# stockeh/swift

Measured on AMD Instinct MI355X. Metric: 6h forecast steps/sec (members x ICs) on 128x256x69 ERA5, higher is better.
Workload: dtype bf16

## Files before the change

### include/swiftk.h

```cpp
#ifndef SWIFTK_H
#define SWIFTK_H

#include <stdint.h>

#ifdef __cplusplus
extern "C" {
#endif

#define SWIFTK_F32 0
#define SWIFTK_BF16 1
#define SWIFTK_BF16X3 2

#define SWIFTK_EINVAL (-1)
#define SWIFTK_ESHAPE (-2)
#define SWIFTK_EALIGN (-3)
#define SWIFTK_EWORKSPACE (-4)

#define SWIFTK_EPI_NONE 0
#define SWIFTK_EPI_BIAS_POS 1
#define SWIFTK_EPI_SWIGLU 2
#define SWIFTK_EPI_QKNORM 3
#define SWIFTK_EPI_SWIGLU_BOTH 6
#define SWIFTK_EPI_SWIGLU_BWD 7
#define SWIFTK_EPI_ACCUM 5
// ... 44 lines not shown
int swiftk_modnorm_residual_pair_slabs_bf16(const void* y_slabs, int64_t ldy, int64_t slab_stride, void* x_hi, int64_t ldh, void* x_lo,
                                            int64_t ldl, int lo_bits, const float* gamma, const float* beta, const float* mod,
                                            int64_t ldmod, int64_t M, int d, int64_t rows_per_sample, float eps, void* stream);
int swiftk_modnorm_residual_pair_halves_bf16(const void* y_slabs, int64_t slab_stride, const int64_t* tail, void* x_hi, int64_t ldh,
                                             void* x_lo, const float* gamma, const float* beta, const float* mod, int64_t ldmod,
                                             int64_t M, int d, int64_t rows_per_sample, float eps, void* stream);
int swiftk_gemm_modnorm_residual_pair(const void* A, int64_t lda, const void* W, int64_t ldw, int64_t K, void* x_hi, int64_t ldh,
                                      void* x_lo, int64_t ldl, const float* gamma, const float* beta, const float* mod,
                                      int64_t ldmod, int64_t M, int d, int64_t rows_per_sample, float eps,
                                      int rows_per_workgroup, void* stream);
int swiftk_split_pair(const float* src, int64_t lds, void* hi, int64_t ldh, void* lo, int64_t ldl, int lo_bits, int64_t rows,
                      int64_t cols, void* stream);
int swiftk_gemm_bias_pos_pair(const void* A, int64_t lda, const void* W, int64_t ldw, void* hi, int64_t ldh, void* lo, int64_t ldl,
                              int64_t M, int64_t N, int64_t K, const float* bias, const float* pos, int64_t pos_rows, void* stream);

int swiftk_patchify(const float* src0, int c0, float s0, const float* src1, int c1, float s1, const float* src2, int c2,
                    float s2, void* A, int64_t lda, int B, int H, int W, int p1, int p2, int dtype, void* stream);
int swiftk_patchify_scaled(const float* src0, int c0, float s0, const float* s0_per_sample, const float* src1, int c1, float s1,
                           const float* src2, int c2, float s2, void* A, int64_t lda, int B, int H, int W, int p1, int p2,
                           int dtype, void* stream);

int swiftk_unpatchify_affine(const float* tok, int64_t ldt, const float* xt, const float* alpha, const float* beta,
                             float* out, int B, int C, int H, int W, int p1, int p2, void* stream);

int swiftk_timestep_embed(const float* t, const float* aux, const float* freqs, const float* aux_w, const float* aux_b,
                          float* emb, int B, int d, int aux_dim, float timestep_weight, void* stream);

int swiftk_linear_small(const float* x, int64_t ldx, const float* W, int64_t ldw, const float* bias, float* out,
                        int64_t ldo, int B, int N, int K, int act, void* stream);

int swiftk_unit_noise(float* out, const int64_t* seeds, const int64_t* step_dev, int64_t step_add, int B,
                      int64_t n_per_unit, int mode, void* stream);
int swiftk_counter_add(int64_t* counter, int64_t value, void* stream);

int swiftk_rollout_update(float* xstd, const float* y, float* phys, const float* mx, const float* sx, const float* st,
                          int B, int C, int64_t hw, void* stream);

int swiftk_unit_checksum(const float* x, double* out, double* scratch, int B, int64_t n, void* stream);

int swiftk_axpby(float* out, float a, const float* x, float b, const float* y, int64_t n, void* stream);

int swiftk_zero_f32(float* p, int64_t n, void* stream);
int swiftk_zero_check_report(unsigned long long* out26);

#define SWIFTK_PROF_ATTENTION 100
int swiftk_profile_gemm(int epilogue, int64_t N);
// ... 227 lines not shown
```

### swift_amd/_lib.py

```python
from __future__ import annotations

import ctypes as C
import os
from typing import Optional

_HERE = os.path.dirname(os.path.abspath(__file__))
LIB_PATH = os.environ.get("SWIFTK_LIB") or os.path.join(_HERE, "csrc", "libswiftk.so")

F32, BF16 = 0, 1
BF16X3 = 2
EPI_NONE, EPI_BIAS_POS, EPI_SWIGLU, EPI_QKNORM, EPI_ACCUM, EPI_SWIGLU_BOTH, EPI_SWIGLU_BWD = 0, 1, 2, 3, 5, 6, 7
EPI_QKNORM_JVP, EPI_SWIGLU_JVP = 8, 9
EPI_SWIGLU_SPLIT3 = 10
ATTN_PRENORM, ATTN_NO_PIPE, ATTN_TILED = 1, 2, 4
PROF_ATTENTION = 100

_ERR = {-1: "SWIFTK_EINVAL (bad argument)", -2: "SWIFTK_ESHAPE (unsupported shape)",
        -3: "SWIFTK_EALIGN (misaligned pointer / leading dimension)", -4: "SWIFTK_EWORKSPACE (workspace too small)"}


class SwiftkError(RuntimeError):
    pass


# ... 44 lines not shown
        + [("layers_host", C.POINTER(Layer))]
        + [("head_dim", C.c_int32)]
    )


_p, _i, _l, _f = C.c_void_p, C.c_int, C.c_int64, C.c_float
_SIGS = {
    "swiftk_version": ([], C.c_int),
    "swiftk_gemm_k_pad": ([_i, _l], _l),
    "swiftk_gemm": ([_p, _l, _p, _l, _p, _l, _l, _l, _l, _i, _i, _i, _p, _p, _l, _p], _i),
    "swiftk_gemm_chunked": ([_p, _l, _p, _l, _p, _l, _l, _l, _l, _i, _i, _i, _p, _p, _l, _i, _p, _l, _p], _i),
    "swiftk_gemm_chunk_scratch_bytes": ([], _l),
    "swiftk_window_attention": ([_p, _l, _p, _l, _p, _i, _i, _i, _i, _i, _i, _i, _i, _i, _p], _i),
    "swiftk_modnorm_residual": ([_p, _l, _p, _p, _l, _p, _p, _p, _l, _l, _i, _l, _f, _i, _p], _i),
    "swiftk_modnorm_residual_pair": ([_p, _l, _p, _l, _p, _l, _i, _p, _p, _p, _l, _l, _i, _l, _f, _p], _i),
    "swiftk_modnorm_residual_pair_to": ([_p, _l, _p, _p, _l, _p, _l, _i, _p, _p, _p, _l, _l, _i, _l, _f, _p], _i),
    "swiftk_modnorm_residual_pair_slabs": ([_p, _l, _l, _p, _l, _p, _l, _i, _p, _p, _p, _l, _l, _i, _l, _f, _p], _i),
    "swiftk_split_pair": ([_p, _l, _p, _l, _p, _l, _i, _l, _l, _p], _i),
    "swiftk_unit_noise": ([_p, _p, _p, _l, _i, _l, _i, _p], _i),
    "swiftk_counter_add": ([_p, _l, _p], _i),
    "swiftk_patchify": ([_p, _i, _f, _p, _i, _f, _p, _i, _f, _p, _l, _i, _i, _i, _i, _i, _i, _p], _i),
    "swiftk_patchify_scaled": ([_p, _i, _f, _p, _p, _i, _f, _p, _i, _f, _p, _l, _i, _i, _i, _i, _i, _i, _p], _i),
    "swiftk_unpatchify_affine": ([_p, _l, _p, _p, _p, _p, _i, _i, _i, _i, _i, _i, _p], _i),
    "swiftk_timestep_embed": ([_p, _p, _p, _p, _p, _p, _i, _i, _i, _f, _p], _i),
    "swiftk_linear_small": ([_p, _l, _p, _l, _p, _p, _l, _i, _i, _i, _i, _p], _i),
    "swiftk_rollout_update": ([_p, _p, _p, _p, _p, _p, _i, _i, _l, _p], _i),
    "swiftk_cast_pad": ([_p, _l, _p, _l, _l, _l, _i, _p], _i),
    "swiftk_split3": ([_p, _l, _p, _l, _l, _l, _i, _p], _i),
    "swiftk_axpby": ([_p, _f, _p, _f, _p, _l, _p], _i),
    "swiftk_zero_f32": ([_p, _l, _p], _i),
    "swiftk_modnorm_residual_split3": ([_p, _l, _p, _p, _l, _p, _l, _p, _p, _p, _l, _l, _i, _l, _f, _p], _i),
    "swiftk_zero_check_report": ([_p], _i),
    "swiftk_unit_checksum": ([_p, _p, _p, _i, _l, _p], _i),
    "swiftk_timestep_embed_jvp": ([_p, _p, _p, _p, _i, _i, _f, _p], _i),
    "swiftk_silu_jvp": ([_p, _p, _p, _p, _l, _p], _i),
    "swiftk_qknorm_jvp": ([_p, _p, _l, _p, _p, _l, _i, _i, _i, _p], _i),
    "swiftk_window_attention_jvp": ([_p, _p, _l, _p, _p, _l, _i, _i, _i, _i, _i, _i, _i, _i, _p], _i),
    "swiftk_modnorm_jvp": ([_p, _p, _l, _p, _p, _p, _p, _l, _p, _p, _p, _p, _l, _l, _i, _l, _f, _i, _p], _i),
    "swiftk_modnorm_jvp_pair": ([_p, _p, _l, _p, _p, _p, _p, _l, _p, _p, _p, _p, _p, _p, _l, _l, _i, _l, _f, _p], _i),
    "swiftk_swiglu_jvp": ([_p, _p, _l, _p, _p, _l, _l, _i, _i, _p], _i),
    "swiftk_gemm_bias_pos_pair": ([_p, _l, _p, _l, _p, _l, _p, _l, _l, _l, _l, _p, _p, _l, _p], _i),
    "swiftk_gemm_splitk_bf16": ([_p, _l, _p, _l, _p, _l, _l, _l, _l, _l, _i, _p], _i),
    "swiftk_gemm_tail_split_bf16": ([_p, _l, _p, _l, _p, _l, _l, _l, _l, _l, _p, _p], _i),
    "swiftk_modnorm_residual_pair_halves_bf16": ([_p, _l, _p, _p, _l, _p, _p, _p, _p, _l, _l, _i, _l, _f, _p], _i),
    "swiftk_modnorm_residual_pair_slabs_bf16": ([_p, _l, _l, _p, _l, _p, _l, _i, _p, _p, _p, _l, _l, _i, _l, _f, _p], _i),
    "swiftk_embed_bwd_sums": ([_p, _l, _p, _p, _p, _l, _l, _i, _l, _p], _i),
# ... 72 lines not shown
```

### swift_amd/csrc/common.h

```cpp
#pragma once
#include <hip/hip_runtime.h>
#include <stdint.h>

#include "../../include/swiftk.h"

typedef __attribute__((ext_vector_type(8))) __bf16 bf16x8;
typedef __attribute__((ext_vector_type(4))) float f32x4;
typedef __attribute__((ext_vector_type(16))) float f32x16;
typedef __attribute__((ext_vector_type(4))) short s16x4;
typedef uint16_t bf16_t;

#define LDS_PTR(p) ((__attribute__((address_space(3))) void*)(p))
#define GLB_PTR(p) ((const __attribute__((address_space(1))) void*)(p))

#define SWIFTK_CHECK_LAUNCH()                         \
    do {                                              \
        hipError_t e__ = hipGetLastError();           \
        if (e__ != hipSuccess) return (int)e__;       \
    } while (0)

__device__ __forceinline__ bf16_t f2bf(float f) {
    __bf16 b = (__bf16)f;
    return __builtin_bit_cast(bf16_t, b);
}
// ... 134 lines not shown
int swiftk_zero_f32_impl(float* p, int64_t n, void* stream, int who);
extern int g_zero_memset;
int swiftk_zero_check_enable();
int swiftk_zero_check_launch(const float* p, int64_t n, void* stream);

bool swiftk_prof_begin(int kind, int n, hipStream_t st);
void swiftk_prof_end(hipStream_t st);
extern int g_fwd_tiled;
extern int g_fwd_fused;
extern int g_x3_exact;
extern int g_fwd_pair;
extern int g_f32_chunk_k;
extern int g_fwd_splitk;
extern int g_attn_bwd_pipe;
extern int g_attn_bwd_fuse;
extern int g_modnorm_bwd_fused;
extern int g_modnorm_jvp_rows;
extern int g_x3_ffsplit;
extern int g_x3_normsplit;
extern int g_x3_qkonly;
extern int g_x3_attnpv;
extern int g_fwd_tail;
extern int g_fwd_pepair;
extern int g_modnorm_nt;
extern int g_persist_wgs;
extern int g_fwd_rownorm;
extern int g_rownorm_dbg;
extern int g_tn_pp;
extern int g_attn_pp;
extern int g_attn_sl;
extern int g_attn_dbg;
```

### swift_amd/csrc/elementwise.hip

```cpp
#include "common.h"
#include <type_traits>

int g_modnorm_nt = 3;

namespace {

__device__ __forceinline__ void load8_nt(const float* p, float (&v)[8]) {
    typedef __attribute__((ext_vector_type(4))) float v4;
    const v4 a = __builtin_nontemporal_load(reinterpret_cast<const v4*>(p));
    const v4 b = __builtin_nontemporal_load(reinterpret_cast<const v4*>(p + 4));
    v[0] = a[0]; v[1] = a[1]; v[2] = a[2]; v[3] = a[3]; v[4] = b[0]; v[5] = b[1]; v[6] = b[2]; v[7] = b[3];
}
__device__ __forceinline__ void store8_nt(float* p, const float (&v)[8]) {
    typedef __attribute__((ext_vector_type(4))) float v4;
    __builtin_nontemporal_store(v4{v[0], v[1], v[2], v[3]}, reinterpret_cast<v4*>(p));
    __builtin_nontemporal_store(v4{v[4], v[5], v[6], v[7]}, reinterpret_cast<v4*>(p + 4));
}

template <typename T, int SLOTS>
__global__ __launch_bounds__(256) void modnorm_kernel(const T* __restrict__ y, int64_t ldy, float* __restrict__ x,
                                                      T* __restrict__ xc, int64_t ldc, const float* __restrict__ gamma,
                                                      const float* __restrict__ beta, const float* __restrict__ mod,
                                                      int64_t ldmod, int64_t M, int d, int64_t rps, float eps, int nt_x) {
    const bool NT_X = nt_x != 0;
// ... 650 lines not shown
    const int F = a.p1 * a.p2 * a.C;
    const int cpr = (int)(a.lda >> 3);
    const int64_t tok0 = ((int64_t)b * a.gh + gy) * a.gw + gxb * 16;
    for (int i = tid; i < 16 * cpr; i += 256) {
        const int tk = i / cpr, fc = i - tk * cpr;
        float v[8];
        int f = 8 * fc;
        int pp = f / a.C, c = f - pp * a.C;
#pragma unroll
        for (int e = 0; e < 8; ++e) {
            float val = 0.f;
            if (f < F) {
                const int i1 = pp / a.p2, i2 = pp - i1 * a.p2;
                val = ptile[(c * a.p1 + i1) * rs + tk * a.p2 + i2];
            }
            v[e] = val;
            ++f;
            if (++c == a.C) { c = 0; ++pp; }
        }
        store8<T>(A + (tok0 + tk) * a.lda + 8 * fc, v);
    }
}

__global__ __launch_bounds__(256) void unpatchify_kernel(const float* __restrict__ tok, int64_t ldt,
                                                         const float* __restrict__ xt, const float* __restrict__ alpha,
                                                         const float* __restrict__ beta, float* __restrict__ out, int B,
                                                         int C, int H, int W, int p1, int p2) {
    const int64_t total = (int64_t)B * C * H * W;
    const int gw = W / p2, gh = H / p1;
    for (int64_t i = (int64_t)blockIdx.x * 256 + threadIdx.x; i < total; i += (int64_t)gridDim.x * 256) {
        const int xw = (int)(i % W);
        int64_t r = i / W;
        const int yh = (int)(r % H);
        r /= H;
        const int c = (int)(r % C);
        const int64_t b = r / C;
        const int gy = yh / p1, i1 = yh - gy * p1, gx = xw / p2, i2 = xw - gx * p2;
        const float f = tok[(b * gh * gw + (int64_t)gy * gw + gx) * ldt + (c * p1 + i1) * p2 + i2];
        const float bb = beta ? beta[b] : 1.0f;
        float o = bb * f;
        if (xt) o = (alpha ? alpha[b] : 0.0f) * xt[i] + o;
        out[i] = o;
    }
}

__global__ __launch_bounds__(256) void unpatchify4_kernel(const float* __restrict__ tok, int64_t ldt,
// ... 517 lines not shown

extern "C" int swiftk_patchify_scaled(const float* src0, int c0, float s0, const float* s0_per_sample, const float* src1, int c1,
                                      float s1, const float* src2, int c2, float s2, void* A, int64_t lda, int B, int H, int W,
                                      int p1, int p2, int dtype, void* stream) {
    if (!A || !src0 || c0 <= 0 || c1 < 0 || c2 < 0 || B <= 0 || p1 <= 0 || p2 <= 0) return SWIFTK_EINVAL;
    if ((c1 > 0 && !src1) || (c2 > 0 && !src2)) return SWIFTK_EINVAL;
    if (H % p1 || W % p2) return SWIFTK_ESHAPE;
    PatchArgs a;
    a.src[0] = src0; a.src[1] = src1 ? src1 : src0; a.src[2] = src2 ? src2 : src0;
    a.cn[0] = c0; a.cn[1] = c1; a.cn[2] = c2;
    a.c0[0] = 0; a.c0[1] = c0; a.c0[2] = c0 + c1;
    if (c1 == 0) a.c0[1] = 1 << 30;
    if (c2 == 0) a.c0[2] = 1 << 30;
    a.sc[0] = s0; a.sc[1] = s1; a.sc[2] = s2;
    a.sc0 = s0_per_sample;
    a.B = B; a.H = H; a.W = W; a.p1 = p1; a.p2 = p2; a.C = c0 + c1 + c2; a.gh = H / p1; a.gw = W / p2;
    a.lda = lda;
    if (lda < (int64_t)p1 * p2 * a.C) return SWIFTK_ESHAPE;
    hipStream_t st = static_cast<hipStream_t>(stream);
    const int rs = 16 * p2 + 4;
    const size_t tile_bytes = (size_t)a.C * p1 * rs * sizeof(float);
    bool aligned = !(a.gw & 15) && !((16 * p2) & 3) && !(W & 3) && !(lda & 7) && !((uintptr_t)A & 15) && tile_bytes <= 64 * 1024;
    for (int k = 0; k < 3; ++k) aligned = aligned && !((uintptr_t)a.src[k] & 15);
    if (aligned && (dtype == SWIFTK_BF16 || dtype == SWIFTK_F32)) {
        const dim3 grid(a.gw / 16, a.gh, B);
        if (dtype == SWIFTK_BF16)
            hipLaunchKernelGGL(patchify_tiled_kernel<bf16_t>, grid, dim3(256), tile_bytes, st, a, static_cast<bf16_t*>(A), rs);
        else
            hipLaunchKernelGGL(patchify_tiled_kernel<float>, grid, dim3(256), tile_bytes, st, a, static_cast<float*>(A), rs);
        SWIFTK_CHECK_LAUNCH();
        return 0;
    }
    const int grid = grid_for((int64_t)B * a.gh * a.gw * lda);
    if (dtype == SWIFTK_BF16)
        hipLaunchKernelGGL(patchify_kernel<bf16_t>, dim3(grid), dim3(256), 0, st, a, static_cast<bf16_t*>(A));
    else if (dtype == SWIFTK_F32)
        hipLaunchKernelGGL(patchify_kernel<float>, dim3(grid), dim3(256), 0, st, a, static_cast<float*>(A));
    else
        return SWIFTK_EINVAL;
    SWIFTK_CHECK_LAUNCH();
    return 0;
}

extern "C" int swiftk_patchify(const float* src0, int c0, float s0, const float* src1, int c1, float s1, const float* src2,
                               int c2, float s2, void* A, int64_t lda, int B, int H, int W, int p1, int p2, int dtype,
                               void* stream) {
// ... 231 lines not shown
```

### swift_amd/csrc/forward.hip

```cpp
#include "common.h"

#include <algorithm>

int g_fwd_tiled = 1;
int g_x3_exact = 17;
int g_fwd_pair = 2;
int g_f32_chunk_k = 256;
int g_fwd_splitk = 2;
int g_fwd_tail = 3;
int g_fwd_pepair = 1;
int g_x3_attnpv = 1;
int g_x3_qkonly = 2;
int g_x3_ffsplit = 1;
int g_fwd_fused = 1;

namespace {

__global__ __launch_bounds__(256) void zero_cols_kernel(char* p, int64_t ld_b, int64_t col0_b, int64_t ncol_b, int64_t rows) {
    const int64_t per = ncol_b >> 2, total = rows * per;
    for (int64_t i = (int64_t)blockIdx.x * 256 + threadIdx.x; i < total; i += (int64_t)gridDim.x * 256) {
        const int64_t r = i / per, c = i - r * per;
        *reinterpret_cast<uint32_t*>(p + r * ld_b + col0_b + 4 * c) = 0u;
    }
}

struct Layout {
    int64_t emb, h1, lat, mod, ape, x, xt, xlo, qkv, att, y, yslab, hmid, tok, kscr, a3, a3h, total;
};

inline int64_t al(int64_t v) { return (v + 255) & ~(int64_t)255; }

bool model_ok(const swiftk_model* m) {
    if (!m || !m->layers_host) return false;
    if (m->dtype != SWIFTK_F32 && m->dtype != SWIFTK_BF16 && m->dtype != SWIFTK_BF16X3) return false;
    if (m->depth <= 0 || m->dim <= 0 || m->heads <= 0 || m->head_dim < 0 || (m->head_dim == 0 && m->dim % m->heads)) return false;
    if (m->H % m->p1 || m->W % m->p2) return false;
// ... 300 lines not shown
            if (halves_norm)
                RUN(swiftk_modnorm_residual_pair_halves_bf16(yslab, SS, nullptr, xT, m->kd, xlo, ly.ln2_g, ly.ln2_b,
                                                             mod + (int64_t)(2 * i + 1) * 2 * d, ldmod, M, d, ntok, 1e-6f, stream));
            else
            RUN(swiftk_modnorm_residual_pair_slabs_bf16(yslab, d, SS, xT, m->kd, xlo, d, lo_bits, ly.ln2_g, ly.ln2_b,
                                                        mod + (int64_t)(2 * i + 1) * 2 * d, ldmod, M, d, ntok, 1e-6f, stream));
            continue;
        }
        if (splitk) {
            RUN(swiftk_gemm_splitk(hmid, m->kmlp, ly.w2_w, m->kmlp, yslab, d, M * d, M, d, m->kmlp, SWIFTK_BF16, 2, stream));
            RUN(swiftk_modnorm_residual_pair_slabs(yslab, d, M * d, xT, m->kd, xlo, d, lo_bits, ly.ln2_g, ly.ln2_b,
                                                   mod + (int64_t)(2 * i + 1) * 2 * d, ldmod, M, d, ntok, 1e-6f, stream));
            continue;
        }
        RUN(G(hmid, m->kmlp, ly.w2_w, y, d, d, m->kmlp, m->mlp, dt, SWIFTK_EPI_NONE, nullptr, nullptr, 0, (x3_exact & 8) != 0));
        if (pair)
            RUN(swiftk_modnorm_residual_pair(y, d, xT, m->kd, xlo, d, lo_bits, ly.ln2_g, ly.ln2_b, mod + (int64_t)(2 * i + 1) * 2 * d, ldmod,
                                             M, d, ntok, 1e-6f, stream));
        else
            RUN(NORM(y, ly.ln2_g, ly.ln2_b, mod + (int64_t)(2 * i + 1) * 2 * d, true));
    }

    const int po4 = (m->out_ch * m->p1 * m->p2 + 3) & ~3;
    RUN(G(xT, m->kd, m->head_w, tok, po4, po4, kdv, d, SWIFTK_F32, SWIFTK_EPI_NONE, nullptr, nullptr, 0, (x3_exact & 32) != 0));
    RUN(swiftk_unpatchify_affine(tok, po4, xt, alpha, beta, out, B, m->out_ch, m->H, m->W, m->p1, m->p2, stream));
    return 0;
}

extern "C" int swiftk_swinv2_forward(const swiftk_model* m, const float* src0, int c0, float s0, const float* src1, int c1,
                                     float s1, const float* src2, int c2, float s2, const float* t, const float* aux,
                                     const float* xt, const float* alpha, const float* beta, float* out, float* logvar,
                                     int B, void* workspace, int64_t workspace_bytes, void* stream) {
    return swiftk_swinv2_forward_scaled(m, src0, c0, s0, nullptr, src1, c1, s1, src2, c2, s2, t, aux, xt, alpha, beta, out, logvar,
                                        B, workspace, workspace_bytes, stream);
}
```

### swift_amd/csrc/gemm.hip

```cpp
#include "common.h"

int g_persist_wgs = 256;

namespace {

template <typename OutT>
__device__ __forceinline__ float swiglu_out(float g, float u) {
    if constexpr (sizeof(OutT) == 4) return g / (1.0f + expf(-g)) * u;
    else return g * __builtin_amdgcn_rcpf(1.0f + __expf(-g)) * u;
}

constexpr int BM = 256;
constexpr int BN = 352;
constexpr int ROWB = 128;
constexpr int A_BYTES = BM * ROWB;
constexpr int B_BYTES = BN * ROWB;
constexpr int STAGE = A_BYTES + B_BYTES;
constexpr int LDS_BYTES = 2 * STAGE;
constexpr int NT = 512;
constexpr int A_PIECES = A_BYTES / 1024;
constexpr int B_PIECES = B_BYTES / 1024;
constexpr int MI = 4, NI = 11;

constexpr int EPI_QKNORM_TILED = 4;
constexpr int EPI_NONE_TAIL = 12;
constexpr int EPI_BIAS_POS_PAIR = 11;

#ifndef SWIFTK_GEMM_INSTR
#define SWIFTK_GEMM_INSTR 0
#endif
#ifndef SWIFTK_X_VMCNT
#define SWIFTK_X_VMCNT 1
#endif
#ifndef SWIFTK_X_PRIO
#define SWIFTK_X_PRIO 1
#endif
#ifndef SWIFTK_X_PF2
#define SWIFTK_X_PF2 1
#endif
#ifndef SWIFTK_X_FEWREADS
#define SWIFTK_X_FEWREADS 0
#endif
#ifndef SWIFTK_X_NOSILU
#define SWIFTK_X_NOSILU 0
#endif
#ifndef SWIFTK_X_POSPERM
#define SWIFTK_X_POSPERM 0
#endif
// ... 282 lines not shown
#pragma unroll
                for (int i = 0; i < MI; ++i) mma_chunk<T>(acc[i][j], wf, xf[i]);
            }
        }
    };

    const int nk = g.K / (ROWB / (int)sizeof(T));
    stage_load(stage0, 0);
    for (int kt = 0; kt < nk; kt += 2) {
        __builtin_amdgcn_s_waitcnt(0x0F70);
        __syncthreads();
        if (kt + 1 < nk) stage_load(stage1, kt + 1);
        compute(stage0);
        if (kt + 1 < nk) {
            __builtin_amdgcn_s_waitcnt(0x0F70);
            __syncthreads();
            if (kt + 2 < nk) stage_load(stage0, kt + 2);
            compute(stage1);
        }
    }

    if constexpr (EPI == SWIFTK_EPI_QKNORM || EPI == EPI_QKNORM_TILED)
        qknorm_tile<NI>(acc, lane, n0 + wn * 176, g.ep0, const_cast<float*>(g.ep1), m0 + wm * 64, g.M, g.N / 88);
    OutT* C = reinterpret_cast<OutT*>(g.C);
#pragma unroll
    for (int i = 0; i < MI; ++i) {
        const int m = m0 + wm * 64 + i * 16 + r16;
        if (m >= g.M) continue;
#pragma unroll
        for (int j = 0; j < NI; ++j) {
            const int nb = n0 + wn * 176 + j * 16 + 4 * (lane >> 4);
            if (nb >= g.N) continue;
            f32x4 v = acc[i][j];
            if constexpr (EPI == SWIFTK_EPI_BIAS_POS) {
                const float4 b = *reinterpret_cast<const float4*>(g.ep0 + nb);
                v[0] += b.x; v[1] += b.y; v[2] += b.z; v[3] += b.w;
                if (g.ep1) {
                    const float4 p = *reinterpret_cast<const float4*>(g.ep1 + (int64_t)(m % g.pos_rows) * g.N + nb);
                    v[0] += p.x; v[1] += p.y; v[2] += p.z; v[3] += p.w;
                }
            }
            if constexpr (EPI == SWIFTK_EPI_SWIGLU) {
                const float h0 = swiglu_out<OutT>(v[0], v[1]);
                const float h1 = swiglu_out<OutT>(v[2], v[3]);
                store2<OutT>(C + (int64_t)m * g.ldc + (nb >> 1), h0, h1);
            } else {
                store4<OutT>(C + (int64_t)m * g.ldc + nb, v[0], v[1], v[2], v[3]);
            }
        }
    }
}


struct TileIter {
    int ntm, ntn, gm;
    int pb, pt;
    __device__ __forceinline__ void coords(int t, int& tm, int& tn) const {
        const int per = gm * ntn;
        const int grp = t / per, r = t - grp * per;
        const int rows = min(gm, ntm - grp * gm);
        tn = r / rows;
        tm = grp * gm + (r - tn * rows);
        if (pb > 1) tm = (tm % pb) * pt + tm / pb;
    }
};

template <typename T, typename OutT, int EPI, int NI, bool PPK, int SL = 0>
__global__ __launch_bounds__(NT) void gemm_kernel_p(GemmArgs g, int ntm, int gm) {
    constexpr bool SLE = (SL & 1) != 0, SLW = (SL & 2) != 0;
    static_assert(SL == 0 || (sizeof(T) == 2 && sizeof(OutT) == 2 && PPK && (EPI == SWIFTK_EPI_NONE || EPI == SWIFTK_EPI_SWIGLU)),
                  "the straight-line forms exist for the bf16 plain and SwiGLU epilogues of the ping-pong kernel only");
    constexpr int WT = 16 * NI;
    constexpr int BN = 2 * WT;
    constexpr int B_BYTES = BN * ROWB;
    constexpr int STAGE = A_BYTES + B_BYTES;
    constexpr int WP = B_BYTES / 1024;
    constexpr int HD = 8 * NI;
    constexpr bool TOUCH = SWIFTK_X_TOUCH > 0 && NI <= 11 && sizeof(T) == 2;
    constexpr bool HPF = SWIFTK_X_HPF > 0 && EPI == SWIFTK_EPI_SWIGLU_BWD && NI <= 11 && sizeof(T) == 2;
    constexpr bool PAIRED = EPI == SWIFTK_EPI_QKNORM_JVP || EPI == SWIFTK_EPI_SWIGLU_JVP;
    constexpr bool PP = PPK && sizeof(T) == 2 && !TOUCH && !HPF && !SWIFTK_GEMM_INSTR;
    static_assert(SL == 0 || PP, "the straight-line forms are written into the ping-pong walk");
    static_assert(SL == 0 || SWIFTK_X_VMCNT, "the straight-line epilogue takes the interior test of the counted store wait");
    __shared__ __attribute__((aligned(16))) char smem[2 * STAGE + (TOUCH || HPF ? 256 : 0)];
    const int lane = threadIdx.x & 63;
    const int wv = __builtin_amdgcn_readfirstlane(threadIdx.x >> 6);
    const int wm = wv >> 1, wn = wv & 1;
#if SWIFTK_X_POSPERM
    const bool posperm = EPI == EPI_BIAS_POS_PAIR && g.ep1 && g.pos_rows >= BM && g.pos_rows % BM == 0 && g.M % g.pos_rows == 0 && g.ksplit == 1;
    const TileIter it{ntm, g.ntn, gm, posperm ? (int)(g.M / g.pos_rows) : 0, posperm ? (int)(g.pos_rows / BM) : 0};
#else
    const TileIter it{ntm, g.ntn, gm, 0, 0};
#endif
// ... 1096 lines not shown
            if (g.ni == 10) hipLaunchKernelGGL((gemm_kernel_p<T, OutT, EPI, 10, false>), dim3(grid), dim3(NT), 0, st, g, ntm, g_group_m);
            else if (g.ni == 12) hipLaunchKernelGGL((gemm_kernel_p<T, OutT, EPI, 12, false>), dim3(grid), dim3(NT), 0, st, g, ntm, g_group_m);
            else hipLaunchKernelGGL((gemm_kernel_p<T, OutT, EPI, 11, false>), dim3(grid), dim3(NT), 0, st, g, ntm, g_group_m);
        } else {
            hipLaunchKernelGGL((gemm_kernel_p<T, OutT, EPI, 11, false>), dim3(grid), dim3(NT), 0, st, g, ntm, g_group_m);
        }
    }
    if (timed) swiftk_prof_end(st);
    SWIFTK_CHECK_LAUNCH();
    return 0;
}

template <int EPI>
int launch_paired(const GemmArgs& g, hipStream_t st) {
    const int ntm = (g.M + BM - 1) / BM;
    constexpr bool W384 = EPI != EPI_BIAS_POS_PAIR;
    if (!W384 && g.ni == 12) return SWIFTK_ESHAPE;
    const bool timed = swiftk_prof_begin(EPI, g.N, st);
    const int ntiles = ntm * g.ntn;
    const int grid = ntiles < g_persist_wgs ? ntiles : g_persist_wgs;
    if (pp_ok(g)) {
        if (g.ni == 10) hipLaunchKernelGGL((gemm_kernel_p<bf16_t, bf16_t, EPI, 10, true>), dim3(grid), dim3(NT), 0, st, g, ntm, g_group_m);
        else if (W384 && g.ni == 12) hipLaunchKernelGGL((gemm_kernel_p<bf16_t, bf16_t, EPI, W384 ? 12 : 11, true>), dim3(grid), dim3(NT), 0, st, g, ntm, g_group_m);
        else hipLaunchKernelGGL((gemm_kernel_p<bf16_t, bf16_t, EPI, 11, true>), dim3(grid), dim3(NT), 0, st, g, ntm, g_group_m);
    } else {
        if (g.ni == 10) hipLaunchKernelGGL((gemm_kernel_p<bf16_t, bf16_t, EPI, 10, false>), dim3(grid), dim3(NT), 0, st, g, ntm, g_group_m);
        else if (W384 && g.ni == 12) hipLaunchKernelGGL((gemm_kernel_p<bf16_t, bf16_t, EPI, W384 ? 12 : 11, false>), dim3(grid), dim3(NT), 0, st, g, ntm, g_group_m);
        else hipLaunchKernelGGL((gemm_kernel_p<bf16_t, bf16_t, EPI, 11, false>), dim3(grid), dim3(NT), 0, st, g, ntm, g_group_m);
    }
    if (timed) swiftk_prof_end(st);
    SWIFTK_CHECK_LAUNCH();
    return 0;
}

template <typename T, typename OutT>
int dispatch_epi(int epi, const GemmArgs& g, hipStream_t st) {
    switch (epi) {
        case SWIFTK_EPI_NONE: return launch<T, OutT, SWIFTK_EPI_NONE>(g, st);
        case SWIFTK_EPI_BIAS_POS: return launch<T, OutT, SWIFTK_EPI_BIAS_POS>(g, st);
        case SWIFTK_EPI_SWIGLU: return launch<T, OutT, SWIFTK_EPI_SWIGLU>(g, st);
        case SWIFTK_EPI_SWIGLU_BWD:
            if constexpr (sizeof(OutT) == 2 && sizeof(T) == 2) return launch<T, OutT, SWIFTK_EPI_SWIGLU_BWD>(g, st);
            return SWIFTK_EINVAL;
        case SWIFTK_EPI_SWIGLU_BOTH:
            if constexpr (sizeof(OutT) == 2 && sizeof(T) == 2) return launch<T, OutT, SWIFTK_EPI_SWIGLU_BOTH>(g, st);
            return SWIFTK_EINVAL;
        case SWIFTK_EPI_ACCUM:
// ... 43 lines not shown
        case 8: g_fwd_fused = value; return 0;
        case 9: g_attn_bwd_pipe = value; return 0;
        case 11: g_x3_exact = value; return 0;
        case 12: g_fwd_pair = value; return 0;
        case 13: g_f32_chunk_k = value; return 0;
        case 14: g_fwd_splitk = value; return 0;
        case 15: g_attn_bwd_fuse = value; return 0;
        case 16: g_modnorm_bwd_fused = value; return 0;
        case 17: g_modnorm_jvp_rows = value; return 0;
        case 18: g_x3_ffsplit = value; return 0;
        case 19: g_fwd_pepair = value; return 0;
        case 20: g_pp = value; return 0;
        case 21: g_attn_pp = value; return 0;
        case 22: g_tn_pp = value; return 0;
        case 23: g_fwd_rownorm = value; return 0;
        case 24: g_rownorm_dbg = value; return 0;
        case 26: g_x3_normsplit = value; return 0;
        case 27: g_x3_qkonly = value; return 0;
        case 28: g_x3_attnpv = value; return 0;
        case 29: g_fwd_tail = value; return 0;
        case 30: g_attn_sl = value & 3; return 0;
        case 31: g_gemm_sl = value & 3; return 0;
        case 32: g_gemm_sl_seen = 0; return 0;
        case 25:
            g_zero_memset = value;
            return (value & 4) ? swiftk_zero_check_enable() : 0;
    }
    return SWIFTK_EINVAL;
}

extern "C" int swiftk_get_tuning(int key) {
    switch (key) {
        case 0: return g_variant;
        case 1: return g_group_m;
        case 2: return g_persist_wgs;
        case 3: return g_dbg;
        case 4: return g_attn_dbg;
        case 5: return g_fwd_tiled;
        case 6: return g_modnorm_nt;
        case 7: return g_stagger_permille;
        case 8: return g_fwd_fused;
        case 9: return g_attn_bwd_pipe;
        case 11: return g_x3_exact;
        case 12: return g_fwd_pair;
        case 13: return g_f32_chunk_k;
        case 14: return g_fwd_splitk;
        case 15: return g_attn_bwd_fuse;
        case 16: return g_modnorm_bwd_fused;
        case 17: return g_modnorm_jvp_rows;
        case 18: return g_x3_ffsplit;
        case 19: return g_fwd_pepair;
        case 20: return g_pp;
        case 21: return g_attn_pp;
        case 22: return g_tn_pp;
        case 23: return g_fwd_rownorm;
        case 25: return g_zero_memset;
        case 26: return g_x3_normsplit;
        case 27: return g_x3_qkonly;
        case 28: return g_x3_attnpv;
        case 29: return g_fwd_tail;
        case 30: return g_attn_sl;
        case 31: return g_gemm_sl;
        case 32: return g_gemm_sl_seen;
    }
    return SWIFTK_EINVAL;
}

extern "C" int swiftk_profile_gemm(int epilogue, int64_t N) {
    g_prof.epilogue = epilogue;
    g_prof.N = (int)N;
    g_prof.used = 0;
    return 0;
}

extern "C" int swiftk_profile_collect(double* total_ms, int64_t* launches) {
    if (!total_ms || !launches) return SWIFTK_EINVAL;
    double tot = 0.0;
    for (int i = 0; i < g_prof.used; ++i) {
        if (hipEventSynchronize(g_prof.ev[2 * i + 1]) != hipSuccess) return SWIFTK_EINVAL;
        float ms = 0.f;
        if (hipEventElapsedTime(&ms, g_prof.ev[2 * i], g_prof.ev[2 * i + 1]) != hipSuccess) return SWIFTK_EINVAL;
        tot += ms;
    }
    *total_ms = tot;
    *launches = g_prof.used;
    g_prof.used = 0;
// ... 169 lines not shown
    g.ldw_b = ldw * 2;
    g.ldc = ldc;
    g.M = (int)(2 * Mh);
    g.N = (int)N;
    g.K = (int)K;
    g.ep0 = scale;
    g.ep1 = epilogue == SWIFTK_EPI_QKNORM_JVP ? rn : static_cast<const float*>(C2);
    g.pos_rows = (int)ldc2;
    g.ni = ni;
    g.ntn = (int)((N + 32 * ni - 1) / (32 * ni));
    g.dbg = g_dbg;
    g.ksplit = 1;
    g.c_split = 0;
    g.batch_a = g.batch_w = g.batch_c = 0;
    g.khalf = khalf;
    g.touch = 0;
    g.stagger = 0;
    g.kscr = nullptr;
    g.kchunk = 0;
    g.t_gh = g.t_gw = g.t_sh = g.t_sw = g.t_heads = 0;
    hipStream_t st = static_cast<hipStream_t>(stream);
    if (epilogue == SWIFTK_EPI_QKNORM_JVP) return launch_paired<SWIFTK_EPI_QKNORM_JVP>(g, st);
    return launch_paired<SWIFTK_EPI_SWIGLU_JVP>(g, st);
}

extern "C" int swiftk_gemm_bias_pos_pair(const void* A, int64_t lda, const void* W, int64_t ldw, void* hi, int64_t ldh, void* lo,
                                         int64_t ldl, int64_t M, int64_t N, int64_t K, const float* bias, const float* pos,
                                         int64_t pos_rows, void* stream) {
    if (!A || !W || !hi || !lo || !bias || M <= 0 || N <= 0 || K <= 0 || (pos && pos_rows <= 0)) return SWIFTK_EINVAL;
    if (M % 8 || N % 16 || K % 64 || lda < K || ldw < K || ldh < N || ldl < N || M > (1 << 30) || N > (1 << 30)) return SWIFTK_ESHAPE;
    if (((uintptr_t)A & 15) || ((uintptr_t)W & 15) || ((uintptr_t)hi & 15) || ((uintptr_t)lo & 15) || ((uintptr_t)bias & 15) ||
        ((uintptr_t)pos & 15) || (lda * 2) % 16 || (ldw * 2) % 16 || ldh % 8 || ldl % 16)
        return SWIFTK_EALIGN;
    const int ni = N % 352 && N % 320 == 0 ? 10 : 11;
    GemmArgs g;
    g.A = static_cast<const char*>(A);
    g.W = static_cast<const char*>(W);
    g.C = static_cast<char*>(hi);
    g.lda_b = lda * 2;
    g.ldw_b = ldw * 2;
    g.ldc = ldh;
    g.M = (int)M;
    g.N = (int)N;
    g.K = (int)K;
    g.ep0 = bias;
    g.ep1 = pos;
// ... 101 lines not shown
```

Baseline: 392.1.

## Fuse head GEMM with unpatchify, add row-group patchify and straight-line bias-pos GEMM

Adds a GEMM epilogue that writes the head projection directly into the unpatchified output image, applying the alpha/beta affine with xt, so the intermediate token buffer and the separate unpatchify kernel are no longer needed. Adds a persistent row-group patchify kernel that prefetches the next group's loads while the current tile is written out. Routes the bias+pos pair GEMM to the straight-line (SL=2) ping-pong variant. All three sit behind a g_fwd_ends bitmask that defaults to enabled. In exchange the fused epilogue's scattered stores and the new code paths may be less efficient than the original separate kernels.

```diff
diff --git a/include/swiftk.h b/include/swiftk.h
--- a/include/swiftk.h
+++ b/include/swiftk.h
@@ -90,6 +90,8 @@
 
 int swiftk_unpatchify_affine(const float* tok, int64_t ldt, const float* xt, const float* alpha, const float* beta,
                              float* out, int B, int C, int H, int W, int p1, int p2, void* stream);
+int swiftk_gemm_unpatchify_affine(const void* A, int64_t lda, const void* W, int64_t ldw, int64_t K, const float* xt,
+                                  const float* alpha, const float* beta, float* out, int B, int C, int H, int Wd, void* stream);
 
 int swiftk_timestep_embed(const float* t, const float* aux, const float* freqs, const float* aux_w, const float* aux_b,
                           float* emb, int B, int d, int aux_dim, float timestep_weight, void* stream);
diff --git a/swift_amd/_lib.py b/swift_amd/_lib.py
--- a/swift_amd/_lib.py
+++ b/swift_amd/_lib.py
@@ -90,6 +90,7 @@
     "swiftk_patchify": ([_p, _i, _f, _p, _i, _f, _p, _i, _f, _p, _l, _i, _i, _i, _i, _i, _i, _p], _i),
     "swiftk_patchify_scaled": ([_p, _i, _f, _p, _p, _i, _f, _p, _i, _f, _p, _l, _i, _i, _i, _i, _i, _i, _p], _i),
     "swiftk_unpatchify_affine": ([_p, _l, _p, _p, _p, _p, _i, _i, _i, _i, _i, _i, _p], _i),
+    "swiftk_gemm_unpatchify_affine": ([_p, _l, _p, _l, _l, _p, _p, _p, _p, _i, _i, _i, _i, _p], _i),
     "swiftk_timestep_embed": ([_p, _p, _p, _p, _p, _p, _i, _i, _i, _f, _p], _i),
     "swiftk_linear_small": ([_p, _l, _p, _l, _p, _p, _l, _i, _i, _i, _i, _p], _i),
     "swiftk_rollout_update": ([_p, _p, _p, _p, _p, _p, _i, _i, _l, _p], _i),
diff --git a/swift_amd/csrc/common.h b/swift_amd/csrc/common.h
--- a/swift_amd/csrc/common.h
+++ b/swift_amd/csrc/common.h
@@ -180,6 +180,8 @@
 extern int g_x3_attnpv;
 extern int g_fwd_tail;
 extern int g_fwd_pepair;
+extern int g_fwd_ends;
+extern int g_fwd_ends_seen;
 extern int g_modnorm_nt;
 extern int g_persist_wgs;
 extern int g_fwd_rownorm;
diff --git a/swift_amd/csrc/elementwise.hip b/swift_amd/csrc/elementwise.hip
--- a/swift_amd/csrc/elementwise.hip
+++ b/swift_amd/csrc/elementwise.hip
@@ -696,6 +696,80 @@
     }
 }
 
+constexpr int PR_NL = 9, PR_NA = 5;
+template <typename T, int NL, int NA>
+__global__ __launch_bounds__(256) void patchify_rows_kernel(PatchArgs a, T* __restrict__ A, int RS, int ngroups) {
+    extern __shared__ __attribute__((aligned(16))) float ptile[];
+    const int tid = threadIdx.x;
+    const int C = a.C, F = 4 * C;
+    const int nload = 16 * C;
+    const int cpr = (int)(a.lda >> 3);
+    const int gpr = a.gw >> 4;
+    const float* sp[NL];
+    int64_t sb[NL];
+    float scs[NL];
+    bool s0[NL];
+    int lo[NL];
+#pragma unroll
+    for (int k = 0; k < NL; ++k) {
+        int i = k * 256 + tid;
+        i = i < nload ? i : nload - 1;
+        const int q = i & 7, i1 = (i >> 3) & 1, c = i >> 4;
+        const int s = c >= a.c0[2] ? 2 : (c >= a.c0[1] ? 1 : 0);
+        sp[k] = a.src[s] + ((int64_t)(c - a.c0[s]) * a.H + i1) * a.W + 4 * q;
+        sb[k] = (int64_t)a.cn[s] * a.H * a.W;
+        scs[k] = a.sc[s];
+        s0[k] = s == 0 && a.sc0;
+        lo[k] = 2 * q * RS + 2 * i1 * C + c;
+    }
+    int ao[NA];
+#pragma unroll
+    for (int t = 0; t < NA; ++t) {
+        const int i = t * 256 + tid, tk = i / cpr;
+        ao[t] = tk * RS + 8 * (i - tk * cpr);
+    }
+    for (int i = tid; i < 16 * ((int)a.lda - F); i += 256) {
+        const int tk = i / ((int)a.lda - F);
+        ptile[tk * RS + F + (i - tk * ((int)a.lda - F))] = 0.f;
+    }
+    float4 v[NL];
+    auto request = [&](int grp) {
+        const int gxb = grp % gpr, r = grp / gpr;
+        const int gy = r % a.gh, b = r / a.gh;
+        const int64_t pix = (int64_t)gy * 2 * a.W + gxb * 32;
+#pragma unroll
+        for (int k = 0; k < NL; ++k)
+            if (k * 256 + tid < nload) v[k] = *reinterpret_cast<const float4*>(sp[k] + (int64_t)b * sb[k] + pix);
+    };
+    int grp = blockIdx.x;
+    if (grp < ngroups) request(grp);
+    for (; grp < ngroups; grp += gridDim.x) {
+        const int b = (grp / gpr) / a.gh;
+        const float f0 = a.sc0 ? a.sc[0] * a.sc0[b] : a.sc[0];
+#pragma unroll
+        for (int k = 0; k < NL; ++k) {
+            if (k * 256 + tid < nload) {
+                const float sc = s0[k] ? f0 : scs[k];
+                float* p = ptile + lo[k];
+                p[0] = v[k].x * sc; p[C] = v[k].y * sc; p[RS] = v[k].z * sc; p[RS + C] = v[k].w * sc;
+            }
+        }
+        if (grp + (int)gridDim.x < ngroups) request(grp + gridDim.x);
+        __syncthreads();
+        T* dst = A + (int64_t)grp * 16 * a.lda;
+#pragma unroll
+        for (int t = 0; t < NA; ++t) {
+            const int i = t * 256 + tid;
+            if (i < 16 * cpr) {
+                float o[8];
+                load8<float>(ptile + ao[t], o);
+                store8<T>(dst + 8 * i, o);
+            }
+        }
+        __syncthreads();
+    }
+}
+
 __global__ __launch_bounds__(256) void unpatchify_kernel(const float* __restrict__ tok, int64_t ldt,
                                                          const float* __restrict__ xt, const float* __restrict__ alpha,
                                                          const float* __restrict__ beta, float* __restrict__ out, int B,
@@ -1259,6 +1333,21 @@
     const size_t tile_bytes = (size_t)a.C * p1 * rs * sizeof(float);
     bool aligned = !(a.gw & 15) && !((16 * p2) & 3) && !(W & 3) && !(lda & 7) && !((uintptr_t)A & 15) && tile_bytes <= 64 * 1024;
     for (int k = 0; k < 3; ++k) aligned = aligned && !((uintptr_t)a.src[k] & 15);
+    if (aligned && (dtype == SWIFTK_BF16 || dtype == SWIFTK_F32) && (g_fwd_ends & 2) && p1 == 2 && p2 == 2 && a.C <= 16 * PR_NL &&
+        lda <= 128 * PR_NA) {
+        const int RS = (int)((lda + 27) / 32 * 32 + 4);
+        const int64_t ngroups = (int64_t)B * a.gh * (a.gw / 16);
+        const int grid = (int)(ngroups < 768 ? ngroups : 768);
+        g_fwd_ends_seen |= 2;
+        if (dtype == SWIFTK_BF16)
+            hipLaunchKernelGGL((patchify_rows_kernel<bf16_t, PR_NL, PR_NA>), dim3(grid), dim3(256), (size_t)16 * RS * sizeof(float), st, a,
+                               static_cast<bf16_t*>(A), RS, (int)ngroups);
+        else
+            hipLaunchKernelGGL((patchify_rows_kernel<float, PR_NL, PR_NA>), dim3(grid), dim3(256), (size_t)16 * RS * sizeof(float), st, a,
+                               static_cast<float*>(A), RS, (int)ngroups);
+        SWIFTK_CHECK_LAUNCH();
+        return 0;
+    }
     if (aligned && (dtype == SWIFTK_BF16 || dtype == SWIFTK_F32)) {
         const dim3 grid(a.gw / 16, a.gh, B);
         if (dtype == SWIFTK_BF16)
diff --git a/swift_amd/csrc/forward.hip b/swift_amd/csrc/forward.hip
--- a/swift_amd/csrc/forward.hip
+++ b/swift_amd/csrc/forward.hip
@@ -12,6 +12,8 @@
 int g_x3_attnpv = 1;
 int g_x3_qkonly = 2;
 int g_x3_ffsplit = 1;
+int g_fwd_ends = 11;
+int g_fwd_ends_seen = 0;
 int g_fwd_fused = 1;
 
 namespace {
@@ -358,6 +360,10 @@
     }
 
     const int po4 = (m->out_ch * m->p1 * m->p2 + 3) & ~3;
+    if (dt == SWIFTK_BF16 && (g_fwd_ends & 1) && m->p1 == 2 && m->p2 == 2 && m->W % 4 == 0) {
+        const int rc = swiftk_gemm_unpatchify_affine(xT, m->kd, m->head_w, m->kd, kdv, xt, alpha, beta, out, B, m->out_ch, m->H, m->W, stream);
+        if (rc != SWIFTK_ESHAPE && rc != SWIFTK_EALIGN) return rc;
+    }
     RUN(G(xT, m->kd, m->head_w, tok, po4, po4, kdv, d, SWIFTK_F32, SWIFTK_EPI_NONE, nullptr, nullptr, 0, (x3_exact & 32) != 0));
     RUN(swiftk_unpatchify_affine(tok, po4, xt, alpha, beta, out, B, m->out_ch, m->H, m->W, m->p1, m->p2, stream));
     return 0;
diff --git a/swift_amd/csrc/gemm.hip b/swift_amd/csrc/gemm.hip
--- a/swift_amd/csrc/gemm.hip
+++ b/swift_amd/csrc/gemm.hip
@@ -24,6 +24,7 @@
 
 constexpr int EPI_QKNORM_TILED = 4;
 constexpr int EPI_NONE_TAIL = 12;
+constexpr int EPI_UNPATCH = 13;
 constexpr int EPI_BIAS_POS_PAIR = 11;
 
 #ifndef SWIFTK_GEMM_INSTR
@@ -352,6 +353,65 @@
 
     if constexpr (EPI == SWIFTK_EPI_QKNORM || EPI == EPI_QKNORM_TILED)
         qknorm_tile<NI>(acc, lane, n0 + wn * 176, g.ep0, const_cast<float*>(g.ep1), m0 + wm * 64, g.M, g.N / 88);
+    if constexpr (EPI == EPI_UNPATCH) {
+        static_assert(sizeof(OutT) == 4 && 4 * NI * 1024 <= STAGE, "four waves' slabs per stage buffer");
+        const float* __restrict__ xt = g.kscr;
+        float* __restrict__ out = reinterpret_cast<float*>(g.C);
+        const int gh = g.t_gh, gw = g.t_gw, Cch = g.t_heads, Wd = 2 * gw;
+        const int64_t plane = (int64_t)(2 * gh) * Wd;
+        __syncthreads();
+        float* slab = reinterpret_cast<float*>((wv < 4 ? stage0 : stage1) + (wv & 3) * (NI * 1024));
+        const int g4 = lane >> 4, q = lane & 7, i1 = (lane >> 3) & 1, cq = lane >> 4;
+        int tk = m0 + wm * 64 + 2 * q;
+        int gx = tk % gw, gy = (tk / gw) % gh, b = (tk / gw) / gh;
+        const int c0 = ((n0 + wn * 176) >> 2) + cq;
+#pragma unroll
+        for (int i = 0; i < MI; ++i) {
+#pragma unroll
+            for (int j = 0; j < NI; ++j) {
+                const f32x4 v = acc[i][j];
+                float* p = slab + j * 256 + g4 * 64 + r16 * 2;
+                *reinterpret_cast<float2*>(p) = make_float2(v[0], v[1]);
+                *reinterpret_cast<float2*>(p + 32) = make_float2(v[2], v[3]);
+            }
+            __builtin_amdgcn_wave_barrier();
+            if (tk < g.M) {
+                const float bb = g.ep1 ? g.ep1[b] : 1.0f;
+                const float aa = g.ep0 ? g.ep0[b] : 0.0f;
+                const int64_t o0 = ((int64_t)b * Cch * (2 * gh) + 2 * gy + i1) * Wd + 2 * gx;
+                constexpr int JH = 4;
+#pragma unroll
+                for (int jh = 0; jh < NI; jh += JH) {
+                    float4 x[JH];
+                    if (xt) {
+#pragma unroll
+                        for (int jj = 0; jj < JH; ++jj)
+                            if (jh + jj < NI && c0 + 4 * (jh + jj) < Cch)
+                                x[jj] = *reinterpret_cast<const float4*>(xt + o0 + (int64_t)(c0 + 4 * (jh + jj)) * plane);
+                    }
+#pragma unroll
+                    for (int jj = 0; jj < JH; ++jj) {
+                        if (jh + jj < NI && c0 + 4 * (jh + jj) < Cch) {
+                            const float4 f = *reinterpret_cast<const float4*>(slab + (jh + jj) * 256 + lane * 4);
+                            float4 o = make_float4(bb * f.x, bb * f.y, bb * f.z, bb * f.w);
+                            if (xt) {
+                                o.x = aa * x[jj].x + o.x; o.y = aa * x[jj].y + o.y; o.z = aa * x[jj].z + o.z; o.w = aa * x[jj].w + o.w;
+                            }
+                            *reinterpret_cast<float4*>(out + o0 + (int64_t)(c0 + 4 * (jh + jj)) * plane) = o;
+                        }
+                    }
+                }
+            }
+            __builtin_amdgcn_wave_barrier();
+            tk += 16;
+            gx += 16;
+            while (gx >= gw) {
+                gx -= gw;
+                if (++gy == gh) { gy = 0; ++b; }
+            }
+        }
+        return;
+    }
     OutT* C = reinterpret_cast<OutT*>(g.C);
 #pragma unroll
     for (int i = 0; i < MI; ++i) {
@@ -398,7 +458,8 @@
 template <typename T, typename OutT, int EPI, int NI, bool PPK, int SL = 0>
 __global__ __launch_bounds__(NT) void gemm_kernel_p(GemmArgs g, int ntm, int gm) {
     constexpr bool SLE = (SL & 1) != 0, SLW = (SL & 2) != 0;
-    static_assert(SL == 0 || (sizeof(T) == 2 && sizeof(OutT) == 2 && PPK && (EPI == SWIFTK_EPI_NONE || EPI == SWIFTK_EPI_SWIGLU)),
+    static_assert(SL == 0 || (sizeof(T) == 2 && sizeof(OutT) == 2 && PPK && (EPI == SWIFTK_EPI_NONE || EPI == SWIFTK_EPI_SWIGLU)) ||
+                      (SL == 2 && sizeof(T) == 2 && sizeof(OutT) == 2 && PPK && EPI == EPI_BIAS_POS_PAIR && NI == 11),
                   "the straight-line forms exist for the bf16 plain and SwiGLU epilogues of the ping-pong kernel only");
     constexpr int WT = 16 * NI;
     constexpr int BN = 2 * WT;
@@ -1541,7 +1602,17 @@
     if (pp_ok(g)) {
         if (g.ni == 10) hipLaunchKernelGGL((gemm_kernel_p<bf16_t, bf16_t, EPI, 10, true>), dim3(grid), dim3(NT), 0, st, g, ntm, g_group_m);
         else if (W384 && g.ni == 12) hipLaunchKernelGGL((gemm_kernel_p<bf16_t, bf16_t, EPI, W384 ? 12 : 11, true>), dim3(grid), dim3(NT), 0, st, g, ntm, g_group_m);
-        else hipLaunchKernelGGL((gemm_kernel_p<bf16_t, bf16_t, EPI, 11, true>), dim3(grid), dim3(NT), 0, st, g, ntm, g_group_m);
+        else {
+            bool walked = false;
+            if constexpr (EPI == EPI_BIAS_POS_PAIR && !SWIFTK_X_POSPERM) {
+                if ((g_fwd_ends & 8) && g.ksplit == 1) {
+                    g_fwd_ends_seen |= 8;
+                    hipLaunchKernelGGL((gemm_kernel_p<bf16_t, bf16_t, EPI, 11, true, 2>), dim3(grid), dim3(NT), 0, st, g, ntm, g_group_m);
+                    walked = true;
+                }
+            }
+            if (!walked) hipLaunchKernelGGL((gemm_kernel_p<bf16_t, bf16_t, EPI, 11, true>), dim3(grid), dim3(NT), 0, st, g, ntm, g_group_m);
+        }
     } else {
         if (g.ni == 10) hipLaunchKernelGGL((gemm_kernel_p<bf16_t, bf16_t, EPI, 10, false>), dim3(grid), dim3(NT), 0, st, g, ntm, g_group_m);
         else if (W384 && g.ni == 12) hipLaunchKernelGGL((gemm_kernel_p<bf16_t, bf16_t, EPI, W384 ? 12 : 11, false>), dim3(grid), dim3(NT), 0, st, g, ntm, g_group_m);
@@ -1631,6 +1702,8 @@
         case 30: g_attn_sl = value & 3; return 0;
         case 31: g_gemm_sl = value & 3; return 0;
         case 32: g_gemm_sl_seen = 0; return 0;
+        case 33: g_fwd_ends = value & 11; return 0;
+        case 34: g_fwd_ends_seen = 0; return 0;
         case 25:
             g_zero_memset = value;
             return (value & 4) ? swiftk_zero_check_enable() : 0;
@@ -1671,6 +1744,8 @@
         case 30: return g_attn_sl;
         case 31: return g_gemm_sl;
         case 32: return g_gemm_sl_seen;
+        case 33: return g_fwd_ends;
+        case 34: return g_fwd_ends_seen;
     }
     return SWIFTK_EINVAL;
 }
@@ -1886,6 +1961,51 @@
     hipStream_t st = static_cast<hipStream_t>(stream);
     if (epilogue == SWIFTK_EPI_QKNORM_JVP) return launch_paired<SWIFTK_EPI_QKNORM_JVP>(g, st);
     return launch_paired<SWIFTK_EPI_SWIGLU_JVP>(g, st);
+}
+
+extern "C" int swiftk_gemm_unpatchify_affine(const void* A, int64_t lda, const void* W, int64_t ldw, int64_t K, const float* xt,
+                                             const float* alpha, const float* beta, float* out, int B, int C, int H, int Wd,
+                                             void* stream) {
+    if (!A || !W || !out || B <= 0 || C <= 0 || H <= 0 || Wd <= 0 || K <= 0) return SWIFTK_EINVAL;
+    if (H % 2 || Wd % 4) return SWIFTK_ESHAPE;
+    const int64_t M = (int64_t)B * (H / 2) * (Wd / 2), N = 4 * (int64_t)C;
+    if (K % 64 == 32 && lda >= K + 32 && ldw >= K + 32) K += 32;
+    if (K % 64 || lda < K || ldw < K || M > (1 << 30) || N > (1 << 30) || K > (1 << 30)) return SWIFTK_ESHAPE;
+    if (!(g_variant == 0 || (M & 7) || (N & 7))) return SWIFTK_ESHAPE;
+    if (((uintptr_t)A & 15) || ((uintptr_t)W & 15) || (lda * 2) % 16 || (ldw * 2) % 16 || ((uintptr_t)out & 15) || ((uintptr_t)xt & 15))
+        return SWIFTK_EALIGN;
+    GemmArgs g;
+    g.A = static_cast<const char*>(A);
+    g.W = static_cast<const char*>(W);
+    g.C = reinterpret_cast<char*>(out);
+    g.lda_b = lda * 2;
+    g.ldw_b = ldw * 2;
+    g.ldc = 0;
+    g.M = (int)M;
+    g.N = (int)N;
+    g.K = (int)K;
+    g.ep0 = alpha;
+    g.ep1 = beta;
+    g.pos_rows = 0;
+    g.ni = NI;
+    g.ntn = (int)((N + BN - 1) / BN);
+    g.dbg = 0;
+    g.ksplit = 1;
+    g.c_split = 0;
+    g.batch_a = g.batch_w = g.batch_c = 0;
+    g.khalf = 0;
+    g.touch = 0;
+    g.stagger = 0;
+    g.tail_from = 0;
+    g.kscr = const_cast<float*>(xt);
+    g.kchunk = 0;
+    g.t_gh = H / 2; g.t_gw = Wd / 2; g.t_sh = g.t_sw = 0; g.t_heads = C;
+    hipStream_t st = static_cast<hipStream_t>(stream);
+    const int ntm = (int)((M + BM - 1) / BM);
+    g_fwd_ends_seen |= 1;
+    hipLaunchKernelGGL((gemm_kernel<bf16_t, float, EPI_UNPATCH>), dim3(ntm * g.ntn), dim3(NT), 0, st, g);
+    SWIFTK_CHECK_LAUNCH();
+    return 0;
 }
 
 extern "C" int swiftk_gemm_bias_pos_pair(const void* A, int64_t lda, const void* W, int64_t ldw, void* hi, int64_t ldh, void* lo,
```

Result: no change. 393.8 (median of 6 runs) (+0.4%).
